# tkonolige/city2ba

Hardware: NVIDIA B200
Metric: camera-point visibility tests/sec (higher is better)
Workload: dtype f64

## Files before the change

city2ba_b200/csrc/c2b_api.cu:

```cuda
#include <algorithm>
#include <charconv>
#include <chrono>
#include <cmath>
#include <cstdlib>
#include <condition_variable>
#include <deque>
#include <mutex>
#include <new>
#include <string>
#include <thread>
#include <vector>

#if defined(__linux__)
#include <cerrno>
#include <fcntl.h>
#include <unistd.h>
#include <sys/mman.h>
#include <sys/stat.h>
#endif

#include "c2b_bal.cuh"
#include "c2b_bal_read.cuh"
#include "c2b_bvh.cuh"
#include "c2b_common.cuh"
// ... 670 lines not shown
}

static void reach_box(const double clo[3], const double chi[3], double max_dist, double lo[3], double hi[3]) {
  for (int k = 0; k < 3; ++k) {
    const double pad = max_dist + 1e-6 * (std::fabs(max_dist) + std::fabs(clo[k]) + std::fabs(chi[k]));
    lo[k] = clo[k] - pad;
    hi[k] = chi[k] + pad;
  }
}

static int build_grid(c2b_ctx *ctx, CtxExtra *x, double max_dist) {
  cudaStream_t st = ctx->stream;
  const uint64_t P = ctx->P;
  C2B_CUDA(cudaStreamSynchronize(st));
  GridDesc g;
  double h = max_dist * x->tun.grid_cell_factor;
  double ext[3];
  for (int k = 0; k < 3; ++k) {
    g.min_c[k] = x->pts_bounds[k];
    g.max_c[k] = x->pts_bounds[3 + k];
    ext[k] = g.max_c[k] - g.min_c[k];
    if (!(ext[k] >= 0.0) || std::isinf(ext[k])) ext[k] = 0.0;
    g.lo[k] = std::isfinite(g.min_c[k]) ? g.min_c[k] : 0.0;
  }
  if (!(h > 0.0) || !std::isfinite(h)) h = 1.0;
  const double max_cells = 4194304.0;
  auto cells_at = [&](double hh) {
    double total = 1.0;
    for (int k = 0; k < 3; ++k) total *= std::min(std::floor(ext[k] / hh) + 1.0, 1e9);
    return total;
  };
  x->grid.hinted = false;
  g.drop = 0;
  for (int k = 0; k < 3; ++k) g.rlo[k] = g.rhi[k] = 0.0;
  bool odd_bounds = false;
  for (int k = 0; k < 3; ++k) odd_bounds = odd_bounds || !std::isfinite(g.min_c[k]) || !std::isfinite(g.max_c[k]);
  if (ctx->C) {
    double clo[3], chi[3], rlo[3], rhi[3];
    C2B_TRY(camera_bbox(ctx, clo, chi));
    reach_box(clo, chi, max_dist, rlo, rhi);
    bool usable = true;
    for (int k = 0; k < 3; ++k) usable = usable && std::isfinite(rlo[k]) && std::isfinite(rhi[k]) && rlo[k] <= rhi[k];
    double frac = 1.0;
    if (usable)
      for (int k = 0; k < 3; ++k) {
        const double a = std::fmax(g.min_c[k], rlo[k]), b = std::fmin(g.max_c[k], rhi[k]);
        if (ext[k] > 0.0) frac *= a <= b ? std::fmin((b - a) / ext[k], 1.0) : 0.0;
      }
    if (usable && (cells_at(h) > max_cells || odd_bounds || frac < 0.7)) {
      for (int k = 0; k < 3; ++k) {
        const double a = std::fmax(g.min_c[k], rlo[k]), b = std::fmin(g.max_c[k], rhi[k]);
        g.lo[k] = a <= b ? a : rlo[k];
        ext[k] = a <= b ? b - a : 0.0;
        g.min_c[k] = g.lo[k];
        g.max_c[k] = a <= b ? b : g.lo[k];
        g.rlo[k] = rlo[k];
        g.rhi[k] = rhi[k];
        x->grid.hint_lo[k] = rlo[k];
        x->grid.hint_hi[k] = rhi[k];
      }
      g.drop = 1;
      x->grid.hinted = true;
    }
  }
  for (;;) {
    double total = 1.0;
    for (int k = 0; k < 3; ++k) {
      double nk = std::floor(ext[k] / h) + 1.0;
      if (nk > 1e9) nk = 1e9;
      g.n[k] = (int)nk;
      total *= nk;
    }
    if (total <= max_cells) break;
    h *= 1.5;
  }
  g.inv_h = 1.0 / h;
  uint64_t n_cells = (uint64_t)g.n[0] * g.n[1] * g.n[2];
  C2B_TRY(ctx->cell_of_pt.ensure(P * 4));
  C2B_TRY(ctx->cell_start.ensure((n_cells + 1) * 4));
  C2B_TRY(ctx->cell_cursor.ensure((n_cells + 1) * 4));
  C2B_TRY(ctx->grid_x.ensure(P * 8));
  C2B_TRY(ctx->grid_y.ensure(P * 8));
  C2B_TRY(ctx->grid_z.ensure(P * 8));
  C2B_TRY(ctx->grid_idx.ensure(P * 4));
  C2B_CUDA(cudaMemsetAsync(ctx->cell_start.p, 0, (n_cells + 1) * 4, st));
  const double *px = ctx->pts.as<double>(), *py = px + P, *pz = py + P;
  k_grid_count<<<blocks_for(P, 256), 256, 0, st>>>(px, py, pz, P, g, ctx->cell_of_pt.as<uint32_t>(),
                                                   ctx->cell_start.as<uint32_t>());
  C2B_KERNEL_CHECK();
  C2B_TRY(exclusive_scan_u32(st, ctx->cell_start.as<uint32_t>(), ctx->cell_start.as<uint32_t>(),
                             n_cells + 1, nullptr, ctx->scan_tmp));
  C2B_CUDA(cudaMemcpyAsync(ctx->cell_cursor.p, ctx->cell_start.p, (n_cells + 1) * 4, cudaMemcpyDeviceToDevice, st));
  k_grid_fill<<<blocks_for(P, 256), 256, 0, st>>>(
      px, py, pz, P, ctx->cell_of_pt.as<uint32_t>(), ctx->cell_cursor.as<uint32_t>(), ctx->grid_x.as<double>(),
      ctx->grid_y.as<double>(), ctx->grid_z.as<double>(), ctx->grid_idx.as<uint32_t>());
  C2B_KERNEL_CHECK();
  x->grid.valid = true;
  x->grid.max_dist = max_dist;
  x->grid.points_version = x->points_version;
  x->grid.desc = g;
  x->grid.n_cells = n_cells;
  return C2B_OK;
}

static int ensure_grid(c2b_ctx *ctx, CtxExtra *x, double max_dist) {
  if (!(ctx->C && ctx->P)) return C2B_OK;
  bool valid = x->grid.valid && x->grid.max_dist == max_dist && x->grid.points_version == x->points_version;
  if (valid && x->grid.hinted && !x->grid_locked) {
    double clo[3], chi[3], rlo[3], rhi[3];
    C2B_TRY(camera_bbox(ctx, clo, chi));
    reach_box(clo, chi, max_dist, rlo, rhi);
    for (int k = 0; k < 3; ++k) valid = valid && rlo[k] >= x->grid.hint_lo[k] && rhi[k] <= x->grid.hint_hi[k];
  }
  if (!valid) C2B_TRY(build_grid(ctx, x, max_dist));
  return C2B_OK;
}

namespace {

void fill_stats(c2b_ctx *ctx, c2b_obs *stats, uint64_t C, uint64_t n_cand, uint64_t pairs_eval,
                uint64_t nodes, uint64_t tris) {
  if (!stats) return;
  memset(stats, 0, sizeof *stats);
  stats->n_cameras = C;
  stats->n_obs = ctx->out_O;
  stats->n_candidates = n_cand;
  stats->pairs_evaluated = pairs_eval;
  stats->nodes_visited = nodes;
  stats->tris_tested = tris;
  auto ms = [&](int a, int b) {
    float t = 0;
    cudaEventElapsedTime(&t, ctx->ev[a], ctx->ev[b]);
    return t;
  };
  stats->ms_prep = ms(EV_H2D, EV_PREP);
  stats->ms_cull = ms(EV_PREP, EV_CULL);
  stats->ms_sort = ms(EV_CULL, EV_SORT);
  stats->ms_traverse = ms(EV_SORT, EV_TRAVERSE);
  stats->ms_compact = ms(EV_TRAVERSE, EV_COMPACT);
  stats->ms_total = ms(EV_START, EV_D2H);
}

int visibility_grid_fused(c2b_ctx *ctx, CtxExtra *x, const c2b_scene *scene, double max_dist,
                          const c2b_vis_options &opt, int pbits, int cbits, c2b_obs *stats) {
  cudaStream_t st = ctx->stream;
  const uint64_t C = ctx->C, P = ctx->P;
  const int sel = ctx->out_sel;
  C2B_TRY(ensure_grid(ctx, x, max_dist));
  C2B_CUDA(cudaEventRecord(ctx->ev[EV_PREP], st));

  C2B_TRY(ctx->counters.ensure(128));
  C2B_TRY(ctx->out_offsets[sel].ensure((C + 1) * 8));
  C2B_CUDA(cudaMemsetAsync(ctx->counters.p, 0, 128, st));
  uint64_t n_cand = 0, pairs_eval = 0, total_obs = 0, nodes = 0, tris_t = 0;
  if (!(C && P)) {
    C2B_CUDA(cudaMemsetAsync(ctx->out_offsets[sel].p, 0, (C + 1) * 8, st));
    for (int e : {EV_CULL, EV_SORT, EV_TRAVERSE, EV_COMPACT, EV_D2H}) C2B_CUDA(cudaEventRecord(ctx->ev[e], st));
    C2B_CUDA(cudaStreamSynchronize(st));
    ctx->out_C = C;
    ctx->out_O = 0;
    x->have_result = true;
    x->res_candidates = 0;
    fill_stats(ctx, stats, C, 0, 0, 0, 0);
    return C2B_OK;
  }

  int parts_log2 = 0;
  {
    const uint64_t warps = (uint64_t)ctx->sm_count * FU_RESIDENT_WARPS;
    if (2 * C <= warps) parts_log2 = 1;
    if (4 * C <= warps) parts_log2 = 2;
    if (x->tun.parts_log2 >= 0) parts_log2 = x->tun.parts_log2;
  }
  const uint64_t slots = C << parts_log2;
  C2B_TRY(ctx->ev_off.ensure((slots + 1) * 4));
  C2B_TRY(ctx->vis_count.ensure((slots + 1) * 4));
  C2B_TRY(ctx->seg_off.ensure((slots + 1) * 4));
  const double *cxp = ctx->cam_center.as<double>();
  const bool mesh = opt.occlusion == C2B_OCC_MESH && scene && scene->n_nodes > 0;
  FusedArgs fa;
  memset(&fa, 0, sizeof fa);
  fa.cams = ctx->cams.as<double>();
  fa.cen_x = cxp;
  fa.cen_y = cxp + C;
  fa.cen_z = cxp + 2 * C;
  fa.C = C;
  fa.gx = ctx->grid_x.as<double>();
  fa.gy = ctx->grid_y.as<double>();
  fa.gz = ctx->grid_z.as<double>();
  fa.gidx = ctx->grid_idx.as<uint32_t>();
  fa.cell_start = ctx->cell_start.as<uint32_t>();
  fa.g = x->grid.desc;
  fa.max_dist = max_dist;
  fa.t_star = exact_sq_threshold(max_dist);
  fa.scene_absmax = scene_abs_max(scene);
  fa.endpoint_guard_rel = opt.endpoint_guard_rel;
  fa.block_length = opt.block_length;
  fa.block_inset = opt.block_inset;
  fa.parts_log2 = parts_log2;
  C2B_TRY(ctx->plan_rows.ensure(C * FU_ROWS * sizeof(uint2)));
  C2B_TRY(ctx->plan_row_count.ensure(C * 4));
  fa.rows = ctx->plan_rows.as<uint2>();
  fa.row_count = ctx->plan_row_count.as<uint32_t>();
  fa.ev_count = ctx->ev_off.as<uint32_t>();
  fa.vis_count = ctx->vis_count.as<uint32_t>();
  fa.counters = ctx->counters.as<unsigned long long>();

  uint32_t *d_total = ctx->counters.as<uint32_t>() + 12;
  uint32_t *d_max = ctx->counters.as<uint32_t>() + 13;
  unsigned long long h_cnt[16];

  cudaStream_t ax = ctx->aux_stream;
  if (mesh) {
    const uint32_t trilist_cap = (uint32_t)x->tun.trilist_cap;
    C2B_TRY(ctx->tri_list.ensure((size_t)C * trilist_cap * 4));
    C2B_TRY(ctx->tri_count.ensure(C * 4));
    float rmax = (float)max_dist;
    if ((double)rmax < max_dist) rmax = std::nextafter(rmax, INFINITY);
    rmax = rmax * (1.0f + 4e-6f);
    fa.nodes = scene->nodes.as<float4>();
    fa.tris = scene->tris.as<float4>();
    fa.n_nodes = (int)scene->n_nodes;
    fa.tri_list = ctx->tri_list.as<uint32_t>();
    fa.tri_count = ctx->tri_count.as<uint32_t>();
    fa.tri_cap = trilist_cap;
    fa.hoist_max = (uint32_t)std::min(x->tun.hoist_max, FU_HOIST);
    fa.packet_bvh = x->tun.packet_bvh;
    const bool tl_warp = x->tun.trilist_warp >= 0 ? x->tun.trilist_warp != 0 : C < 32768;
    C2B_CUDA(cudaEventRecord(ctx->ev_fork, st));
    C2B_CUDA(cudaStreamWaitEvent(ax, ctx->ev_fork, 0));
    if (tl_warp)
      k_cam_trilist_warp<<<blocks_for(C, TL_WARPS), TL_WARPS * 32, 0, ax>>>(
          fa.nodes, fa.n_nodes, fa.cen_x, fa.cen_y, fa.cen_z, C, rmax, fa.scene_absmax, trilist_cap,
          ctx->tri_list.as<uint32_t>(), ctx->tri_count.as<uint32_t>(), fa.counters + 0);
    else
      k_cam_trilist<<<blocks_for(C, 128), 128, 0, ax>>>(fa.nodes, fa.n_nodes, fa.cen_x, fa.cen_y, fa.cen_z, C, rmax,
                                                       fa.scene_absmax, trilist_cap, ctx->tri_list.as<uint32_t>(),
                                                       ctx->tri_count.as<uint32_t>(), fa.counters + 0);
    C2B_KERNEL_CHECK();
    C2B_CUDA(cudaEventRecord(ctx->ev_join, ax));
  }
  k_cam_plan<<<blocks_for(C + 1, 128), 128, 0, st>>>(fa);
  C2B_KERNEL_CHECK();
  C2B_TRY(exclusive_scan_u32(st, fa.ev_count, fa.ev_count, slots + 1, nullptr, ctx->scan_tmp));
  if (mesh) C2B_CUDA(cudaStreamWaitEvent(st, ctx->ev_join, 0));
  const uint64_t max_pairs = x->tun.max_pairs;
  const bool mt = mesh && opt.predicate == C2B_PRED_MT;
  const bool optimistic = x->tun.optimistic && x->memo.valid && !opt.count_traversal && ctx->scratch_idx.cap >= 4 &&
                          ctx->out_idx[sel].cap >= 4 && ctx->out_uv[sel].cap >= 16;
  bool any_overflow = x->memo.any_overflow;
  if (!optimistic) {
    C2B_TRY(read_counters(ctx, h_cnt));
    pairs_eval = h_cnt[1];
    any_overflow = h_cnt[0] != 0;
    if (pairs_eval >= max_pairs)
      return set_error(ERR_TOO_LARGE, "more than 2^32 camera-point pairs inside max_dist in one call; shard the cameras");
    C2B_TRY(ctx->scratch_idx.ensure(std::max<uint64_t>(pairs_eval, 1) * 4));
  }
  fa.scratch_idx = ctx->scratch_idx.as<uint32_t>();
  fa.scratch_cap = ctx->scratch_idx.cap / 4;
  C2B_CUDA(cudaEventRecord(ctx->ev[EV_CULL], st));
  C2B_CUDA(cudaEventRecord(ctx->ev[EV_SORT], st));

  C2B_CUDA(cudaMemsetAsync(ctx->vis_count.p, 0, (slots + 1) * 4, st));
  {
    const unsigned nb = (unsigned)std::min<uint64_t>(blocks_for(slots, FU_WARPS), (uint64_t)ctx->sm_count * 8), nt = FU_WARPS * 32;
    const bool cnt = opt.count_traversal != 0;
    if (mt) {
      k_visibility_fused<FU_OCC_NONE, false, 3, false><<<nb, nt, 0, st>>>(fa);
    } else if (mesh) {
      if (cnt)
        k_visibility_fused<FU_OCC_MESH, true, 3, true><<<nb, nt, 0, st>>>(fa);
      else if (any_overflow)
// ... 2009 lines not shown
```

city2ba_b200/csrc/c2b_common.cuh:

```cuda
#pragma once
#include <cuda_runtime.h>

#include <atomic>
#include <cstdarg>
#include <cstdint>
#include <cstdio>
#include <cstring>
#include <memory>
#include <string>
#include <type_traits>
#include <utility>
#include <vector>
#if defined(__linux__)
#include <sys/syscall.h>
#include <unistd.h>
#endif

#include "../../include/city2ba_cuda.h"

namespace c2b {

inline std::string &last_error_ref() {
  static thread_local std::string s;
  return s;
// ... 138 lines not shown
  template <class T>
  T *as() const {
    return reinterpret_cast<T *>(p);
  }
};

template <class H, cudaError_t (*make)(H *, unsigned), cudaError_t (*destroy)(H)>
class CudaHandle {
 public:
  CudaHandle() = default;
  CudaHandle(CudaHandle &&o) noexcept : h_(std::exchange(o.h_, nullptr)) {}
  CudaHandle &operator=(CudaHandle &&o) noexcept {
    if (this != &o) {
      release();
      h_ = std::exchange(o.h_, nullptr);
    }
    return *this;
  }
  ~CudaHandle() { release(); }
  int create(unsigned flags = 0) {
    release();
    C2B_CUDA(make(&h_, flags));
    return C2B_OK;
  }
  void release() {
    if (h_) destroy(h_);
    h_ = nullptr;
  }
  operator H() const { return h_; }

 private:
  H h_ = nullptr;
};
using Event = CudaHandle<cudaEvent_t, cudaEventCreateWithFlags, cudaEventDestroy>;
using Stream = CudaHandle<cudaStream_t, cudaStreamCreateWithFlags, cudaStreamDestroy>;

static_assert(!std::is_copy_constructible<DevBuf>::value && !std::is_copy_constructible<PinBuf>::value &&
                  !std::is_copy_constructible<Event>::value && !std::is_copy_constructible<Stream>::value,
              "owners of device resources are move-only");

struct CtxExtra;

enum StageEvent {
  EV_START = 0,
  EV_H2D,
  EV_PREP,
  EV_CULL,
  EV_SORT,
  EV_TRAVERSE,
  EV_COMPACT,
  EV_D2H,
  EV_COUNT
};

}

struct c2b_scene {
  int device = 0;
  uint64_t n_tris = 0;
  uint64_t n_nodes = 0;
  float lo[3] = {0, 0, 0}, hi[3] = {0, 0, 0};
  c2b::DevBuf nodes;
  c2b::DevBuf tris;
};

struct c2b_ctx {
  int device = 0;
  int sm_count = 148;
  c2b::Stream stream;
  c2b::Stream copy_stream;
  c2b::Stream aux_stream;
  std::unique_ptr<c2b::CtxExtra> extra;
  c2b::Event ev[c2b::EV_COUNT];

  uint64_t C = 0, P = 0;
  c2b::DevBuf cams_all;
  c2b::DevBuf cams;
  c2b::DevBuf cam_center;
  c2b::DevBuf pts;
  c2b::DevBuf pts_aos;
  c2b::DevBuf stage;
  c2b::PinBuf pin_in;

  c2b::DevBuf cell_of_pt, cell_start, cell_cursor, grid_x, grid_y, grid_z, grid_idx;

  c2b::DevBuf pool_key, pool_uv, cam_count, counters;
  c2b::DevBuf sort_keys[2], sort_vals[2], sort_hist;
  c2b::DevBuf scan_tmp[3];
  uint64_t pool_capacity = 0;

  c2b::DevBuf vis_words, word_prefix;
  c2b::DevBuf out_offsets[2], out_idx[2], out_uv[2];
  int out_sel = 0;
  uint64_t out_C = 0, out_O = 0;
  c2b::Event ev_fork, ev_join;
  c2b::Event ev_ready[2], ev_copied[2];
  c2b::DevBuf misc;
  c2b::DevBuf tri_list, tri_count;
  c2b::DevBuf ev_off, vis_count, seg_off, scratch_idx, plan_rows, plan_row_count;
  int numa_node = -1;

  c2b::DevBuf nz_cams, nz_centers, nz_pts, nz_uv, nz_scratch;
  float noise_ms[3] = {0, 0, 0};

  c2b::DevBuf pr_cams[2], pr_pts[2], pr_off[2], pr_idx[2], pr_uv[2];
  c2b::DevBuf pr_parent, pr_size, pr_cam_cnt, pr_pt_cnt, pr_words, pr_prefix, pr_small;

  c2b::PinBuf h_offsets, h_idx, h_uv, h_small;

  ~c2b_ctx();
};
```

city2ba_b200/csrc/c2b_cull.cuh:

```cuda
#pragma once
#include "c2b_common.cuh"
#include "c2b_math.cuh"

namespace c2b {

struct CullArgs {
  const double *cams;
  const double *cen_x, *cen_y, *cen_z;
  const double *px, *py, *pz;
  uint64_t C, P;
  double t_star;
  double t_cons;
  int pbits;
  uint64_t *pool_key;
  double2 *pool_uv;
  uint32_t *cam_count;
  unsigned long long *counters;
  uint64_t pool_capacity;
};

constexpr uint64_t POOL_SENTINEL = ~0ull;

__global__ void k_cam_prep(const double *__restrict__ cams, uint64_t C, double *__restrict__ cx,
                           double *__restrict__ cy, double *__restrict__ cz) {
// ... 87 lines not shown
#pragma unroll
  for (int k = 0; k < CB_PPT; ++k) {
    pi[k] = (uint64_t)blockIdx.x * (CB_THREADS * CB_PPT) + (uint64_t)k * CB_THREADS + threadIdx.x;
    bool ok = pi[k] < a.P;
    px[k] = ok ? a.px[pi[k]] : 1e300;
    py[k] = ok ? a.py[pi[k]] : 1e300;
    pz[k] = ok ? a.pz[pi[k]] : 1e300;
  }
  __syncthreads();
  uint2 *q = s_q[warp];
  int qn = 0;
  const double tc = a.t_cons;
  for (int j = 0; j < ncam; ++j) {
    const double cx = s_cx[j], cy = s_cy[j], cz = s_cz[j];
    bool pass[CB_PPT];
    bool any = false;
#pragma unroll
    for (int k = 0; k < CB_PPT; ++k) {
      double dx = px[k] - cx, dy = py[k] - cy, dz = pz[k] - cz;
      double d2 = fma(dz, dz, fma(dy, dy, dx * dx));
      pass[k] = d2 < tc;
      any |= pass[k];
    }
    if (__any_sync(0xffffffffu, any)) {
#pragma unroll
      for (int k = 0; k < CB_PPT; ++k) {
        unsigned m = __ballot_sync(0xffffffffu, pass[k]);
        if (m) {
          if (pass[k]) q[qn + __popc(m & ((1u << lane) - 1u))] = make_uint2((uint32_t)(cam0 + j), (uint32_t)pi[k]);
          qn += __popc(m);
          __syncwarp();
          if (qn >= 32) {
            brute_drain(a, q, qn - 32, 32);
            qn -= 32;
            __syncwarp();
          }
        }
      }
    }
  }
  if (qn > 0) brute_drain(a, q, 0, qn);
}

struct GridDesc {
  double lo[3];
  double inv_h;
  int n[3];
  int drop;
  double max_c[3];
  double min_c[3];
  double rlo[3], rhi[3];
};

__device__ __forceinline__ int grid_coord(const GridDesc &g, int k, double x) {
  double t = floor(dmul(dsub(x, g.lo[k]), g.inv_h));
  int c = t < 0.0 ? 0 : (t >= (double)g.n[k] ? g.n[k] - 1 : (int)t);
  if (!(t == t)) c = 0;
  return c;
}

__global__ void __launch_bounds__(256) k_grid_count(const double *__restrict__ px, const double *__restrict__ py,
                                                    const double *__restrict__ pz, uint64_t P, GridDesc g,
                                                    uint32_t *__restrict__ cell_of_pt, uint32_t *__restrict__ cell_count) {
  const uint64_t i = (uint64_t)blockIdx.x * blockDim.x + threadIdx.x;
  const int lane = threadIdx.x & 31;
  uint32_t cell = 0xffffffffu;
  if (i < P) {
    const double x = px[i], y = py[i], z = pz[i];
    const bool out = g.drop && (x < g.rlo[0] || x > g.rhi[0] || y < g.rlo[1] || y > g.rhi[1] || z < g.rlo[2] || z > g.rhi[2]);
    if (!out) {
      int cx = grid_coord(g, 0, x), cy = grid_coord(g, 1, y), cz = grid_coord(g, 2, z);
      cell = ((uint32_t)cz * g.n[1] + cy) * g.n[0] + cx;
    }
    cell_of_pt[i] = cell;
  }
  const unsigned peers = __match_any_sync(0xffffffffu, cell);
  if (cell != 0xffffffffu && lane == __ffs(peers) - 1) atomicAdd(&cell_count[cell], (uint32_t)__popc(peers));
}

__global__ void __launch_bounds__(256) k_grid_fill(const double *__restrict__ px, const double *__restrict__ py,
                                                   const double *__restrict__ pz, uint64_t P,
                                                   const uint32_t *__restrict__ cell_of_pt, uint32_t *__restrict__ cursor,
                                                   double *__restrict__ gx, double *__restrict__ gy,
                                                   double *__restrict__ gz, uint32_t *__restrict__ gidx) {
  const uint64_t i = (uint64_t)blockIdx.x * blockDim.x + threadIdx.x;
  const int lane = threadIdx.x & 31;
  const uint32_t cell = i < P ? cell_of_pt[i] : 0xffffffffu;
  const bool valid = cell != 0xffffffffu;
  double x = 0.0, y = 0.0, z = 0.0;
  if (valid) {
    x = px[i];
    y = py[i];
    z = pz[i];
  }
  const unsigned peers = __match_any_sync(0xffffffffu, cell);
  const int leader = __ffs(peers) - 1;
  uint32_t first = 0;
  if (valid && lane == leader) first = atomicAdd(&cursor[cell], (uint32_t)__popc(peers));
  const uint32_t pos = __shfl_sync(0xffffffffu, first, leader) + __popc(peers & ((1u << lane) - 1u));
  if (valid) {
    gx[pos] = x;
    gy[pos] = y;
    gz[pos] = z;
    gidx[pos] = (uint32_t)i;
  }
}

__global__ void k_pts_bounds_partial(const double *__restrict__ px, const double *__restrict__ py,
                                     const double *__restrict__ pz, uint64_t P,
                                     double *__restrict__ partial ) {
  double lo[3] = {INFINITY, INFINITY, INFINITY}, hi[3] = {-INFINITY, -INFINITY, -INFINITY};
  for (uint64_t i = (uint64_t)blockIdx.x * blockDim.x + threadIdx.x; i < P;
       i += (uint64_t)gridDim.x * blockDim.x) {
    double v[3] = {px[i], py[i], pz[i]};
#pragma unroll
    for (int k = 0; k < 3; ++k) {
      lo[k] = fmin(lo[k], v[k]);
      hi[k] = fmax(hi[k], v[k]);
    }
  }
  __shared__ double s[6][8];
#pragma unroll
  for (int k = 0; k < 3; ++k) {
#pragma unroll
    for (int o = 16; o > 0; o >>= 1) {
      lo[k] = fmin(lo[k], __shfl_xor_sync(0xffffffffu, lo[k], o));
      hi[k] = fmax(hi[k], __shfl_xor_sync(0xffffffffu, hi[k], o));
    }
    if ((threadIdx.x & 31) == 0) {
      s[k][threadIdx.x >> 5] = lo[k];
      s[3 + k][threadIdx.x >> 5] = hi[k];
    }
  }
  __syncthreads();
  if (threadIdx.x < 6) {
    double r = s[threadIdx.x][0];
    for (int w = 1; w < (int)(blockDim.x >> 5); ++w)
      r = threadIdx.x < 3 ? fmin(r, s[threadIdx.x][w]) : fmax(r, s[threadIdx.x][w]);
    partial[6 * (uint64_t)blockIdx.x + threadIdx.x] = r;
  }
}
__global__ void k_pts_bounds_final(const double *__restrict__ partial, int nb, double *__restrict__ out) {
  const int lane = threadIdx.x & 31;
  double lo[3] = {INFINITY, INFINITY, INFINITY}, hi[3] = {-INFINITY, -INFINITY, -INFINITY};
  for (int b = lane; b < nb; b += 32) {
#pragma unroll
    for (int k = 0; k < 3; ++k) {
      lo[k] = fmin(lo[k], partial[6 * b + k]);
      hi[k] = fmax(hi[k], partial[6 * b + 3 + k]);
    }
  }
#pragma unroll
  for (int k = 0; k < 3; ++k) {
#pragma unroll
    for (int o = 16; o > 0; o >>= 1) {
      lo[k] = fmin(lo[k], __shfl_xor_sync(0xffffffffu, lo[k], o));
      hi[k] = fmax(hi[k], __shfl_xor_sync(0xffffffffu, hi[k], o));
    }
  }
  if (lane == 0) {
#pragma unroll
    for (int k = 0; k < 3; ++k) {
      out[k] = lo[k];
      out[3 + k] = hi[k];
    }
  }
}

}
```

city2ba_b200/csrc/c2b_fused.cuh:

```cuda
#pragma once
#include "c2b_common.cuh"
#include "c2b_compact.cuh"
#include "c2b_cull.cuh"
#include "c2b_math.cuh"
#include "c2b_traverse.cuh"

namespace c2b {

struct FusedArgs {
  const double *cams;
  const double *cen_x, *cen_y, *cen_z;
  uint64_t C;
  const double *gx, *gy, *gz;
  const uint32_t *gidx;
  const uint32_t *cell_start;
  GridDesc g;
  double max_dist;
  double t_star;
  const float4 *nodes;
  const float4 *tris;
  int n_nodes;
  float scene_absmax;
  const uint32_t *tri_list;
  const uint32_t *tri_count;
  uint32_t tri_cap;
  uint32_t hoist_max;
  int packet_bvh;
  int endpoint_guard_rel;
  double block_length, block_inset;
  int parts_log2;
  uint2 *rows;
  uint32_t *row_count;
  uint32_t *ev_count;
  uint32_t *scratch_idx;
  uint64_t scratch_cap;
  uint32_t *vis_count;
  unsigned long long *counters;
};
enum { FU_FLAG_SCRATCH = 1, FU_FLAG_NEED_WALK = 2, FU_FLAG_OUT = 4 };

__device__ __forceinline__ bool camera_cell_range(const GridDesc &g, const double cc[3], double max_dist,
                                                  int lo[3], int hi[3]) {
  bool empty = !(max_dist > 0.0);
#pragma unroll
  for (int k = 0; k < 3; ++k) {
    const double eps = dadd(dmul(1e-9, dadd(fabs(cc[k]), fabs(max_dist))), 1e-300);
    const double a0 = dsub(dsub(cc[k], max_dist), eps), a1 = dadd(dadd(cc[k], max_dist), eps);
    if (a0 > g.max_c[k] || a1 < g.min_c[k]) empty = true;
    lo[k] = grid_coord(g, k, a0);
    hi[k] = grid_coord(g, k, a1);
  }
  if (!(cc[0] == cc[0] && cc[1] == cc[1] && cc[2] == cc[2])) empty = true;
  return !empty;
}


__device__ __forceinline__ bool trim_halfspace(const GridDesc &g, double cell_h, double nx, double ny, double nz,
                                               double off, double xr, double mag_floor, double y0, double y1,
                                               double z0, double z1, int &x0, int &x1) {
  const double my = ny == 0.0 ? 0.0 : dmul(ny, ny > 0.0 ? y0 : y1);
  const double mz = nz == 0.0 ? 0.0 : dmul(nz, nz > 0.0 ? z0 : z1);
  const double bmin = dadd(dadd(my, mz), off);
  const double mag = dadd(dadd(dadd(dadd(fabs(my), fabs(mz)), fabs(off)), xr), mag_floor);
  if (bmin == bmin && fabs(bmin) < INFINITY) {
    const double slack = dadd(dmul(1e-9, mag), 1e-300);
    if (xr <= slack) {
      if (bmin > dmul(2.0, slack)) return false;
    } else {
      const double xlim = ddiv(-dsub(bmin, slack), nx);
      if (xlim == xlim) {
        const double xs = dmul(1e-9, dadd(fabs(xlim), cell_h));
        if (nx > 0.0) {
          const double xe = dadd(xlim, xs);
          if (xe < g.lo[0]) return false;
          const int xc = grid_coord(g, 0, xe);
          x1 = xc < x1 ? xc : x1;
        } else {
          const double xe = dsub(xlim, xs);
          if (xe > g.max_c[0]) return false;
          const int xc = grid_coord(g, 0, xe);
          x0 = xc > x0 ? xc : x0;
        }
        if (x0 > x1) return false;
      }
    }
  }
  return true;
}

constexpr int FU_ROWS = 32;
constexpr uint32_t FU_ROWS_MANY = 0xffffffffu;

struct RowRange {
  uint32_t start, end;
};

__device__ __forceinline__ RowRange camera_row(const GridDesc &g, const uint32_t *__restrict__ cell_start,
// ... 1 lines not shown
                                               const int lo[3], const int hi[3], double cell_h, int y, int z) {
  RowRange r{0u, 0u};
  int x0 = lo[0], x1 = hi[0];
  const double sl = dmul(1e-6, cell_h);
  const double y0 = y == 0 ? g.min_c[1] : dsub(dadd(g.lo[1], dmul((double)y, cell_h)), sl);
  const double y1 = y == g.n[1] - 1 ? g.max_c[1] : dadd(dadd(g.lo[1], dmul((double)(y + 1), cell_h)), sl);
  const double z0 = z == 0 ? g.min_c[2] : dsub(dadd(g.lo[2], dmul((double)z, cell_h)), sl);
  const double z1 = z == g.n[2] - 1 ? g.max_c[2] : dadd(dadd(g.lo[2], dmul((double)(z + 1), cell_h)), sl);
  const double reach = dadd(fabs(cc[0]), fabs(max_dist));
  {
    const double dy = fmax(fmax(dsub(y0, cc[1]), dsub(cc[1], y1)), 0.0);
    const double dz = fmax(fmax(dsub(z0, cc[2]), dsub(cc[2], z1)), 0.0);
    const double rem = dsub(dmul(dmul(max_dist, max_dist), 1.000000001), dadd(dmul(dy, dy), dmul(dz, dz)));
    if (rem < 0.0) return r;
    if (rem == rem && rem < INFINITY) {
      const double w = dadd(dmul(dsqrt(rem), 1.000000001), dmul(1e-9, reach));
      const double xa = dsub(cc[0], w), xb = dadd(cc[0], w);
      if (xa > g.max_c[0] || xb < g.min_c[0]) return r;
      const int ca = grid_coord(g, 0, xa), cb = grid_coord(g, 0, xb);
      x0 = ca > x0 ? ca : x0;
      x1 = cb < x1 ? cb : x1;
      if (x0 > x1) return r;
    }
  }
  const double f = c[12];
  const bool planar_image = c[13] == 0.0 && c[14] == 0.0 && fabs(f) < INFINITY;
  double rmax = 0.0;
#pragma unroll
  for (int k = 0; k < 12; ++k) rmax = fmax(rmax, fabs(c[k]));
  const double span = dadd(dadd(dadd(fabs(cc[0]), fabs(cc[1])), fabs(cc[2])), dmul(3.0, fabs(max_dist)));
  const double mag_floor = dmul(dadd(planar_image ? fabs(f) : 0.0, 1.0), dmul(rmax, dadd(span, 1.0)));
  if (!trim_halfspace(g, cell_h, c[2], c[5], c[8], c[11], dmul(fabs(c[2]), reach), mag_floor, y0, y1, z0, z1, x0, x1))
    return r;
  if (planar_image) {
#pragma unroll
    for (int k = 0; k < 4; ++k) {
      const int row = k >> 1;
      const double sf = (k & 1) ? -f : f;
      const double nx = dadd(dmul(sf, c[row]), c[2]), ny = dadd(dmul(sf, c[3 + row]), c[5]);
      const double nz = dadd(dmul(sf, c[6 + row]), c[8]), off = dadd(dmul(sf, c[9 + row]), c[11]);
      if (!trim_halfspace(g, cell_h, nx, ny, nz, off, dmul(fabs(nx), reach), mag_floor, y0, y1, z0, z1, x0, x1))
        return r;
    }
  }
  const uint32_t rowbase = ((uint32_t)z * g.n[1] + y) * g.n[0];
  r.start = cell_start[rowbase + x0];
  r.end = cell_start[rowbase + x1 + 1];
  return r;
}

__device__ __forceinline__ bool cull_predicate(const double *cam, V3 center, V3 p, double t_star) {
  const V3 d{dsub(center.x, p.x), dsub(center.y, p.y), dsub(center.z, p.z)};
  if (!(mag2(d) < t_star)) return false;
  const double pcz = dadd(dadd(dadd(dmul(cam[2], p.x), dmul(cam[5], p.y)), dmul(cam[8], p.z)), cam[11]);
  if (!(pcz <= 0.0)) return false;
  const double pcx = dadd(dadd(dadd(dmul(cam[0], p.x), dmul(cam[3], p.y)), dmul(cam[6], p.z)), cam[9]);
  const double pcy = dadd(dadd(dadd(dmul(cam[1], p.x), dmul(cam[4], p.y)), dmul(cam[7], p.z)), cam[10]);
  const double f = cam[12], k1 = cam[13], k2 = cam[14];
  const double az = fabs(pcz);
  if (az > 1e-30 && az < 1e30) {
    const double iz = (double)__frcp_rn(__double2float_rn(pcz));
    const double a = pcx * iz, b = pcy * iz;
    double ua, va, bu, bv;
    if (k1 == 0.0 && k2 == 0.0) {
      ua = fabs(f * a);
      va = fabs(f * b);
      bu = 2e-6 * ua;
      bv = 2e-6 * va;
    } else {
      const double m2p = a * a + b * b;
      const double r = 1.0 + k1 * m2p + k2 * (m2p * m2p);
      const double rb = 1.0 + fabs(k1) * m2p + fabs(k2) * (m2p * m2p);
      ua = fabs(f * r * a);
      va = fabs(f * r * b);
      bu = 2e-6 * fabs(f * a) * rb;
      bv = 2e-6 * fabs(f * b) * rb;
    }
    if (ua <= 1.0 - bu && va <= 1.0 - bv) return true;
    if (ua > 1.0 + bu || va > 1.0 + bv) return false;
  }
  double u, v;
  project(f, k1, k2, V3{pcx, pcy, pcz}, u, v);
  return u >= -1.0 && u <= 1.0 && v >= -1.0 && v <= 1.0;
}

__device__ __noinline__ RowRange camera_row_call(const GridDesc &g, const uint32_t *__restrict__ cell_start,
                                                 const double *c, const double *cc, double max_dist, const int *lo,
                                                 const int *hi, double cell_h, int y, int z) {
  return camera_row(g, cell_start, c, cc, max_dist, lo, hi, cell_h, y, z);
}

__global__ void __launch_bounds__(128, 5) k_cam_plan(FusedArgs a) {
  const uint64_t cam = (uint64_t)blockIdx.x * blockDim.x + threadIdx.x;
  const int S = 1 << a.parts_log2;
  unsigned long long n0 = 0, n1 = 0, n2 = 0, n3 = 0;
  if (cam < a.C) {
    const double cc[3] = {a.cen_x[cam], a.cen_y[cam], a.cen_z[cam]};
    int lo[3], hi[3];
    a.row_count[cam] = 0u;
    if (camera_cell_range(a.g, cc, a.max_dist, lo, hi)) {
      double c[15];
#pragma unroll
      for (int k = 0; k < 15; ++k) c[k] = a.cams[15 * cam + k];
      const double cell_h = ddiv(1.0, a.g.inv_h);
      const int nrows = (hi[1] - lo[1] + 1) * (hi[2] - lo[2] + 1);
      const bool keep = nrows <= FU_ROWS;
      a.row_count[cam] = keep ? (uint32_t)nrows : FU_ROWS_MANY;
      int ri = 0;
      for (int z = lo[2]; z <= hi[2]; ++z)
        for (int y = lo[1]; y <= hi[1]; ++y, ++ri) {
          const RowRange rr = camera_row(a.g, a.cell_start, c, cc, a.max_dist, lo, hi, cell_h, y, z);
          if (keep) a.rows[cam * FU_ROWS + ri] = make_uint2(rr.start, rr.end);
          if (rr.end > rr.start) {
            const unsigned long long m = rr.end - rr.start;
            int part = 0;
            for (int q = 1; q < S; ++q)
              if (ri >= (nrows * q) >> a.parts_log2) part = q;
            n0 += part == 0 ? m : 0ull;
            n1 += part == 1 ? m : 0ull;
            n2 += part == 2 ? m : 0ull;
            n3 += part == 3 ? m : 0ull;
          }
        }
    }
    uint32_t *out = a.ev_count + (cam << a.parts_log2);
    out[0] = (uint32_t)n0;
    if (S > 1) out[1] = (uint32_t)n1;
    if (S > 2) {
      out[2] = (uint32_t)n2;
      out[3] = (uint32_t)n3;
    }
  }
  if (cam == a.C) a.ev_count[cam << a.parts_log2] = 0u;
  unsigned long long n = n0 + n1 + n2 + n3;
#pragma unroll
  for (int o = 16; o > 0; o >>= 1) n += __shfl_xor_sync(0xffffffffu, n, o);
  if ((threadIdx.x & 31) == 0 && n) atomicAdd(&a.counters[1], n);
}

struct SortWriteArgs {
  const uint32_t *ev_off;
  const uint32_t *seg_off;
  uint64_t C;
  const uint32_t *scratch_idx;
  const double *cams;
  const double *p_aos;
  uint64_t *out_offsets;
  uint32_t *out_idx;
  double2 *out_uv;
  int key_bits;
  int parts_log2;
  uint64_t out_cap;
  unsigned long long *flags;
};

struct CamSlices {
  uint32_t base, n;
  uint32_t sub[4], eo[4];
};
template <bool MULTI>
__device__ __forceinline__ CamSlices cam_slices(const SortWriteArgs &s, uint64_t cam) {
  CamSlices cs;
  if (!MULTI) {
    cs.base = s.seg_off[cam];
    cs.n = s.seg_off[cam + 1] - cs.base;
    cs.sub[0] = 0u;
// ... 340 lines not shown
  }
  for (uint32_t base = 0; base < n_list; base += 32) {
    const uint32_t j = base + lane;
    bool overlap = false;
    int slot = 0;
    if (j < n_list) {
      const uint32_t node = mylist[j];
      const float4 lo = __ldg(&a.nodes[2 * node]);
      const float4 hi = __ldg(&a.nodes[2 * node + 1]);
      overlap = box_meets_packet(pb, lo, hi);
      slot = __float_as_int(hi.w);
    }
    if (COUNT) n_vis += min(32u, n_list - base);
    if (!test_leaf_chunk<COUNT>(a, pb, slot, overlap, ray, am, ox, oy, oz, rec, lane, n_tri)) break;
  }
  return alive && !((am >> lane) & 1u);
}

constexpr int FU_LIFO = 576;

template <bool COUNT>
__device__ __forceinline__ int packet_bvh_hit(const FusedArgs &a, const Ray &ray, bool have, float ox, float oy,
                                              float oz, float4 *region, int lane, unsigned &n_vis,
                                              unsigned &n_tri) {
  const bool alive = have && (ray.tfar >= 0.0f) && (ray.dx == ray.dx) && (ray.dy == ray.dy) && (ray.dz == ray.dz);
  unsigned am = __ballot_sync(0xffffffffu, alive);
  if (am == 0u) return 0;
  const PacketBounds pb = packet_bounds(ray, alive, ox, oy, oz, a.scene_absmax);
  float4 *rec = region;
  uint32_t *pending = reinterpret_cast<uint32_t *>(region + 96);
  uint32_t *lifo = pending + 64;
  int sp = 1, np = 0;
  if (lane == 0) lifo[0] = 0u;
  __syncwarp();
  while (sp > 0 || np > 0) {
    if (sp > 0 && np <= 32) {
      const int take = sp < 32 ? sp : 32;
      const bool mine = lane < take;
      bool leaf = false, inner = false;
      int slot = 0;
      uint32_t node = 0, right = 0;
      if (mine) {
        node = lifo[sp - take + lane];
        const float4 lo = __ldg(&a.nodes[2 * node]);
        const float4 hi = __ldg(&a.nodes[2 * node + 1]);
        if (box_meets_packet(pb, lo, hi)) {
          slot = __float_as_int(hi.w);
          leaf = slot >= 0;
          inner = !leaf;
          right = (uint32_t)(-slot - 1);
        }
      }
      __syncwarp();
      sp -= take;
      if (COUNT) n_vis += take;
      const unsigned lm = __ballot_sync(0xffffffffu, leaf), im = __ballot_sync(0xffffffffu, inner);
      if (sp + 2 * __popc(im) > FU_LIFO) return 2;
      const unsigned lt = (1u << lane) - 1u;
      if (leaf) pending[np + __popc(lm & lt)] = (uint32_t)slot;
      if (inner) {
        const int pos = sp + 2 * __popc(im & lt);
        lifo[pos] = node + 1u;
        lifo[pos + 1] = right;
      }
      np += __popc(lm);
      sp += 2 * __popc(im);
      __syncwarp();
    } else {
      const int cnt = np < 32 ? np : 32;
      const bool want = lane < cnt;
      const int slot = want ? (int)pending[np - cnt + lane] : 0;
      np -= cnt;
      if (!test_leaf_chunk<COUNT>(a, pb, slot, want, ray, am, ox, oy, oz, rec, lane, n_tri)) break;
    }
  }
  return alive && !((am >> lane) & 1u) ? 1 : 0;
}

constexpr int FU_REGION_F4 = 4 * FU_HOIST;

template <bool MESH>
struct alignas(16) FuWarpSmem {
  float4 rec[MESH ? FU_REGION_F4 : 1];
  double cam[16];
  uint32_t stage[FU_STAGE];
};

template <int OCC, bool COUNT, int MIN_CTAS, bool WALK>
__global__ void __launch_bounds__(FU_WARPS * 32, fu_min_ctas(MIN_CTAS)) k_visibility_fused(FusedArgs a) {
  typedef FuWarpSmem<OCC == FU_OCC_MESH> WarpSmem;
  __shared__ WarpSmem s_w[FU_WARPS];
  const int lane = threadIdx.x & 31, warp = threadIdx.x >> 5;
  uint32_t w_s = (uint32_t)__cvta_generic_to_shared(&s_w[warp]);
  asm volatile("" : "+r"(w_s));
  WarpSmem *const w = reinterpret_cast<WarpSmem *>(__cvta_shared_to_generic((size_t)w_s));
  double *const c = w->cam;
  uint32_t *stage = w->stage;
  unsigned long long found_total = 0;
  unsigned n_vis_nodes = 0, n_tri = 0;
  const double cell_h = ddiv(1.0, a.g.inv_h);
  for (;;) {
    unsigned long long ticket = 0;
    if (lane == 0) ticket = atomicAdd(&a.counters[7], 1ull);
    const uint64_t slot = __shfl_sync(0xffffffffu, ticket, 0);
    const uint64_t cam = slot >> a.parts_log2;
    if (cam >= a.C) break;
    const int part = (int)(slot & ((1u << a.parts_log2) - 1u));
    __syncwarp();
    double creg = 0.0;
    if (lane < 15) creg = __ldg(&a.cams[15 * cam + lane]);
    const V3 cen{a.cen_x[cam], a.cen_y[cam], a.cen_z[cam]};
    const uint32_t planned_rows = a.row_count[cam];
    const uint32_t ev0 = a.ev_count[slot], ev1 = a.ev_count[slot + 1];
    const uint2 myrow = a.rows[cam * FU_ROWS + lane];
    uint32_t n_list = 0, l0 = 0, l1 = 0;
    const uint32_t *mylist = nullptr;
    if (OCC == FU_OCC_MESH) {
      n_list = a.tri_count[cam];
      mylist = a.tri_list + cam * a.tri_cap;
      if ((uint32_t)lane < a.tri_cap) l0 = mylist[lane];
      if ((uint32_t)lane + 32u < a.tri_cap) l1 = mylist[lane + 32];
    }
    if (lane < 15) c[lane] = creg;
    __syncwarp();
    const bool misfit = (uint64_t)ev1 > a.scratch_cap || (OCC == FU_OCC_MESH && !WALK && n_list == TRILIST_OVERFLOW);
    if (misfit && lane == 0)
      atomicOr(&a.counters[12], (unsigned long long)((uint64_t)ev1 > a.scratch_cap ? FU_FLAG_SCRATCH : FU_FLAG_NEED_WALK));
    if (planned_rows == 0u || misfit) {
      if (lane == 0) a.vis_count[slot] = 0;
      continue;
    }
    const float ox = d2f(cen.x), oy = d2f(cen.y), oz = d2f(cen.z);
    const bool hoisted = OCC == FU_OCC_MESH && n_list <= a.hoist_max;
    if (hoisted) hoist_records(a, l0, l1, n_list, ox, oy, oz, w->rec, lane);
    uint32_t *out = a.scratch_idx + ev0;
    const uint32_t out_cap = ev1 - ev0;
    uint32_t nvis = 0;
    int qn = 0, head = 0;

    auto resolve = [&](int count) {
      const bool have = lane < count;
      Ray ray;
      ray.ox = ox; ray.oy = oy; ray.oz = oz;
      ray.dx = ray.dy = ray.dz = 1.0f;
      ray.tfar = -1.0f;
      uint32_t pt = 0;
      V3 p{0.0, 0.0, 0.0};
      if (have) {
        const int e = (head + lane) & (FU_STAGE - 1);
        const uint32_t i = stage[e];
        pt = a.gidx[i];
        p = V3{a.gx[i], a.gy[i], a.gz[i]};
        if (OCC == FU_OCC_MESH) ray = make_ray(cen, p, a.endpoint_guard_rel != 0);
      }
      bool occ = false;
      if (OCC == FU_OCC_MESH) {
        if (WALK && n_list == TRILIST_OVERFLOW) {
          const int r = a.packet_bvh ? packet_bvh_hit<COUNT>(a, ray, have, ox, oy, oz, w->rec, lane, n_vis_nodes, n_tri) : 2;
          occ = r == 2 ? warp_any_hit<COUNT>(a.nodes, a.tris, a.n_nodes, ray, have, a.scene_absmax, a.counters)
                       : r == 1;
        } else
          occ = packet_any_hit<COUNT>(a, mylist, n_list, ray, have, ox, oy, oz, w->rec, hoisted, lane, n_vis_nodes, n_tri);
      } else if (OCC == FU_OCC_ANALYTIC) {
        occ = have && hits_building(cen, p, a.block_length, a.block_inset);
      }
      const bool vis = have && !occ;
      const unsigned m = __ballot_sync(0xffffffffu, vis);
      if (vis) {
        const uint32_t pos = nvis + __popc(m & ((1u << lane) - 1u));
        if (pos < out_cap)
          out[pos] = pt;
        else
          a.counters[5] = 1ull;
      }
      nvis += __popc(m);
    };

    int lo[3] = {0, 0, 0}, hi[3] = {0, 0, 0}, ny = 1, nrows = (int)planned_rows;
    double cc[3] = {cen.x, cen.y, cen.z};
    if (planned_rows == FU_ROWS_MANY) {
      camera_cell_range(a.g, cc, a.max_dist, lo, hi);
      ny = hi[1] - lo[1] + 1;
      nrows = ny * (hi[2] - lo[2] + 1);
    }
    const int row0 = (nrows * part) >> a.parts_log2, row1 = (nrows * (part + 1)) >> a.parts_log2;
    for (int rb = planned_rows != FU_ROWS_MANY ? 0 : row0; rb < row1; rb += 32) {
      RowRange rr{0u, 0u};
      const int ri = rb + lane;
      if (ri >= row0 && ri < row1) {
        if (planned_rows != FU_ROWS_MANY) {
          rr.start = myrow.x;
          rr.end = myrow.y;
        } else {
          rr = camera_row_call(a.g, a.cell_start, c, cc, a.max_dist, lo, hi, cell_h, lo[1] + ri % ny, lo[2] + ri / ny);
        }
      }
      unsigned live = __ballot_sync(0xffffffffu, rr.end > rr.start);
      if (live == 0u) continue;
      int j = __ffs(live) - 1;
      live &= live - 1;
      uint32_t base = __shfl_sync(0xffffffffu, rr.start, j), end = __shfl_sync(0xffffffffu, rr.end, j);
      V3 pn{0.0, 0.0, 0.0};
      if (base + lane < end) pn = V3{a.gx[base + lane], a.gy[base + lane], a.gz[base + lane]};
      for (;;) {
        uint32_t nbase = base + 32, nend = end;
        bool more = true;
        if (nbase >= end) {
          if (live) {
            j = __ffs(live) - 1;
            live &= live - 1;
            nbase = __shfl_sync(0xffffffffu, rr.start, j);
            nend = __shfl_sync(0xffffffffu, rr.end, j);
          } else {
            more = false;
          }
        }
        const uint32_t i = base + lane;
        const V3 pcur = pn;
        if (more && nbase + lane < nend) pn = V3{a.gx[nbase + lane], a.gy[nbase + lane], a.gz[nbase + lane]};
        bool pass = false;
        if (i < end) pass = cull_predicate(c, cen, pcur, a.t_star);
        const unsigned m = __ballot_sync(0xffffffffu, pass);
        if (m != 0u) {
          if (pass) {
            const int e = (head + qn + __popc(m & ((1u << lane) - 1u))) & (FU_STAGE - 1);
            stage[e] = i;
          }
          qn += __popc(m);
          __syncwarp();
          if (qn >= 32) {
            resolve(32);
            __syncwarp();
            head = (head + 32) & (FU_STAGE - 1);
            qn -= 32;
            found_total += 32;
          }
        }
        if (!more) break;
        base = nbase;
        end = nend;
      }
    }
    if (qn > 0) {
      resolve(qn);
      found_total += qn;
    }
    nvis = nvis < out_cap ? nvis : out_cap;
    if (lane == 0) a.vis_count[slot] = nvis;
  }
  if (lane == 0) {
    if (found_total) atomicAdd(&a.counters[4], found_total);
    if (COUNT) {
      atomicAdd(&a.counters[2], (unsigned long long)n_vis_nodes);
      atomicAdd(&a.counters[3], (unsigned long long)n_tri);
    }
  }
}

template <int MIN_CTAS, bool MULTI>
__global__ void __launch_bounds__(SW_WARPS * 32, MIN_CTAS) k_sort_write(SortWriteArgs s) {
  __shared__ uint32_t s_sorted[SW_WARPS][SW_WARP_MAX + SW_WARP_MAX / 32];
  __shared__ uint32_t s_hist[SW_WARPS][SW_BINS];
  __shared__ double s_cam[SW_WARPS][16];
  const int lane = threadIdx.x & 31, warp = threadIdx.x >> 5;
  const uint64_t cam = (uint64_t)blockIdx.x * SW_WARPS + warp;
  if (cam >= s.C) return;
  CamSlices cs = cam_slices<MULTI>(s, cam);
  cs.n = __reduce_max_sync(0xffffffffu, cs.n);
  const uint32_t base = cs.base, n = cs.n;
  if (lane == 0) {
    s.out_offsets[cam] = base;
    if (cam == s.C - 1) s.out_offsets[s.C] = s.seg_off[s.C << s.parts_log2];
  }
  if (n == 0 || n > SW_WARP_MAX) return;
  if ((uint64_t)base + n > s.out_cap) {
    if (lane == 0) atomicOr(s.flags, (unsigned long long)FU_FLAG_OUT);
    return;
  }
  uint32_t *sorted = s_sorted[warp];
  if (n <= 128)
    sort_warp_to_smem<4, MULTI>(s, cs, lane, sorted, s_hist[warp]);
  else if (n <= 256)
    sort_warp_to_smem<8, MULTI>(s, cs, lane, sorted, s_hist[warp]);
  else if (n <= 512)
    sort_warp_to_smem<16, MULTI>(s, cs, lane, sorted, s_hist[warp]);
  else if (n <= 768)
    sort_warp_to_smem<24, MULTI>(s, cs, lane, sorted, s_hist[warp]);
  else
    sort_warp_to_smem<32, MULTI>(s, cs, lane, sorted, s_hist[warp]);
  __syncwarp();
  double *crec = s_cam[warp];
  if (lane < 15) crec[lane] = __ldg(&s.cams[15 * cam + lane]);
  __syncwarp();
  uint32_t c_s = (uint32_t)__cvta_generic_to_shared(crec);
  struct Pt {
    uint32_t idx;
    double x, y, z;
  };
  auto gather = [&](uint32_t k) {
    Pt q{0u, 0.0, 0.0, 0.0};
    if (k < n) {
      q.idx = sorted[sw_pad(k)];
      const double *p = s.p_aos + 3 * (uint64_t)q.idx;
      q.x = __ldg(p);
// ... 84 lines not shown
```

Baseline: 293200 billion.

## Add conservative f32 cull prefilter with packed float4 point layout

Stores a packed float4 (x,y,z as f32 plus the point index) per grid point. The hot cull loop now streams these 16-byte records and runs an f32 classifier using per-camera error bounds, computed once per warp, that decide definite inside or outside. Only ambiguous points fall back to the exact f64 predicate. This is meant to cut f64 arithmetic and the three 8-byte loads per candidate on a GPU with weak FP64 throughput. In exchange it adds a 16-byte-per-point buffer, extra work in grid_fill and per-camera setup, and relies on the error bounds being correct to keep results exact.

```diff
diff --git a/city2ba_b200/csrc/c2b_api.cu b/city2ba_b200/csrc/c2b_api.cu
--- a/city2ba_b200/csrc/c2b_api.cu
+++ b/city2ba_b200/csrc/c2b_api.cu
@@ -776,7 +776,7 @@
   C2B_TRY(ctx->grid_x.ensure(P * 8));
   C2B_TRY(ctx->grid_y.ensure(P * 8));
   C2B_TRY(ctx->grid_z.ensure(P * 8));
-  C2B_TRY(ctx->grid_idx.ensure(P * 4));
+  C2B_TRY(ctx->grid_p4.ensure(P * 16));
   C2B_CUDA(cudaMemsetAsync(ctx->cell_start.p, 0, (n_cells + 1) * 4, st));
   const double *px = ctx->pts.as<double>(), *py = px + P, *pz = py + P;
   k_grid_count<<<blocks_for(P, 256), 256, 0, st>>>(px, py, pz, P, g, ctx->cell_of_pt.as<uint32_t>(),
@@ -787,7 +787,7 @@
   C2B_CUDA(cudaMemcpyAsync(ctx->cell_cursor.p, ctx->cell_start.p, (n_cells + 1) * 4, cudaMemcpyDeviceToDevice, st));
   k_grid_fill<<<blocks_for(P, 256), 256, 0, st>>>(
       px, py, pz, P, ctx->cell_of_pt.as<uint32_t>(), ctx->cell_cursor.as<uint32_t>(), ctx->grid_x.as<double>(),
-      ctx->grid_y.as<double>(), ctx->grid_z.as<double>(), ctx->grid_idx.as<uint32_t>());
+      ctx->grid_y.as<double>(), ctx->grid_z.as<double>(), ctx->grid_p4.as<float4>());
   C2B_KERNEL_CHECK();
   x->grid.valid = true;
   x->grid.max_dist = max_dist;
@@ -882,7 +882,7 @@
   fa.gx = ctx->grid_x.as<double>();
   fa.gy = ctx->grid_y.as<double>();
   fa.gz = ctx->grid_z.as<double>();
-  fa.gidx = ctx->grid_idx.as<uint32_t>();
+  fa.gp = ctx->grid_p4.as<float4>();
   fa.cell_start = ctx->cell_start.as<uint32_t>();
   fa.g = x->grid.desc;
   fa.max_dist = max_dist;
diff --git a/city2ba_b200/csrc/c2b_common.cuh b/city2ba_b200/csrc/c2b_common.cuh
--- a/city2ba_b200/csrc/c2b_common.cuh
+++ b/city2ba_b200/csrc/c2b_common.cuh
@@ -244,7 +244,7 @@
   c2b::DevBuf stage;
   c2b::PinBuf pin_in;
 
-  c2b::DevBuf cell_of_pt, cell_start, cell_cursor, grid_x, grid_y, grid_z, grid_idx;
+  c2b::DevBuf cell_of_pt, cell_start, cell_cursor, grid_x, grid_y, grid_z, grid_p4;
 
   c2b::DevBuf pool_key, pool_uv, cam_count, counters;
   c2b::DevBuf sort_keys[2], sort_vals[2], sort_hist;
diff --git a/city2ba_b200/csrc/c2b_cull.cuh b/city2ba_b200/csrc/c2b_cull.cuh
--- a/city2ba_b200/csrc/c2b_cull.cuh
+++ b/city2ba_b200/csrc/c2b_cull.cuh
@@ -193,7 +193,7 @@
                                                    const double *__restrict__ pz, uint64_t P,
                                                    const uint32_t *__restrict__ cell_of_pt, uint32_t *__restrict__ cursor,
                                                    double *__restrict__ gx, double *__restrict__ gy,
-                                                   double *__restrict__ gz, uint32_t *__restrict__ gidx) {
+                                                   double *__restrict__ gz, float4 *__restrict__ gp) {
   const uint64_t i = (uint64_t)blockIdx.x * blockDim.x + threadIdx.x;
   const int lane = threadIdx.x & 31;
   const uint32_t cell = i < P ? cell_of_pt[i] : 0xffffffffu;
@@ -213,7 +213,7 @@
     gx[pos] = x;
     gy[pos] = y;
     gz[pos] = z;
-    gidx[pos] = (uint32_t)i;
+    gp[pos] = make_float4(d2f(x), d2f(y), d2f(z), __uint_as_float((uint32_t)i));
   }
 }
 
diff --git a/city2ba_b200/csrc/c2b_fused.cuh b/city2ba_b200/csrc/c2b_fused.cuh
--- a/city2ba_b200/csrc/c2b_fused.cuh
+++ b/city2ba_b200/csrc/c2b_fused.cuh
@@ -12,7 +12,7 @@
   const double *cen_x, *cen_y, *cen_z;
   uint64_t C;
   const double *gx, *gy, *gz;
-  const uint32_t *gidx;
+  const float4 *gp;
   const uint32_t *cell_start;
   GridDesc g;
   double max_dist;
@@ -180,6 +180,66 @@
   double u, v;
   project(f, k1, k2, V3{pcx, pcy, pcz}, u, v);
   return u >= -1.0 && u <= 1.0 && v >= -1.0 && v <= 1.0;
+}
+
+struct CullF32 {
+  float4 c;
+  float4 rx;
+  float4 ry;
+  float4 rz;
+};
+
+__device__ __noinline__ void cull_f32_constants(const double *cam, V3 cen, double t_star, CullF32 *out) {
+  const double u = 5.9604644775390625e-08, w = 1.1102230246251565e-16;
+  const double cm = fmax(fmax(fabs(cen.x), fabs(cen.y)), fabs(cen.z));
+  double rmax = 0.0;
+  for (int k = 0; k < 12; ++k) rmax = fmax(rmax, fabs(cam[k]));
+  const double f = cam[12];
+  const bool dist_ok = cm <= 1e30 && rmax <= 1e30 && t_star >= 1e-30 && t_star <= 1e30;
+  const bool planar = cam[13] == 0.0 && cam[14] == 0.0 && fabs(f) >= 1e-6 && fabs(f) <= 1e6;
+  float tin = -1.0f, tout = __int_as_float(0x7fffffff), kk = INFINITY;
+  if (dist_ok) {
+    const double a = 2.5 * u, b = 2.5 * u * cm + 1e-37, s3b = 1.7320508075688774 * b * (1.0 + 1e-12);
+    const double r = sqrt(t_star);
+    const double ri = (1.0 - a) * r * (1.0 - 1e-12) - s3b, ro = (1.0 + a) * r * (1.0 + 1e-12) + s3b;
+    if (ri > 0.0) tin = __double2float_rd(ri * ri * (1.0 - 4.0 * u) * (1.0 - 1e-12));
+    if (!(tin >= 1e-30f)) tin = -1.0f;
+    tout = __double2float_ru(ro * ro * (1.0 + 4.0 * u) * (1.0 + 1e-12));
+    if (planar && tin > 0.0f) {
+      const double qb = sqrt((double)tout * (1.0 + 4.0 * u)) * (1.0 + 1e-12);
+      const double L = (qb + s3b) / (1.0 - a) * (1.0 + 1e-12);
+      double e[3], mx[3];
+      for (int row = 0; row < 3; ++row) {
+        const double r0 = cam[row], r1 = cam[3 + row], r2 = cam[6 + row], t = cam[9 + row];
+        const double n1 = fabs(r0) + fabs(r1) + fabs(r2);
+        const double tau = fabs(r0 * cen.x + r1 * cen.y + r2 * cen.z + t) + 4.01 * w * (n1 * cm + fabs(t));
+        const double e64 = 4.01 * w * (n1 * (cm + L) + fabs(t));
+        e[row] = (n1 * (4.02 * u * qb + a * L + b) + tau + e64) * (1.0 + 1e-12);
+        mx[row] = (n1 * L + tau + e64) * (1.0 + 1e-12);
+      }
+      const double af = fabs(f), exy = fmax(e[0], e[1]), xmax = fmax(mx[0], mx[1]);
+      const double k0 = af * exy + u * af * (xmax + exy) + e[2] + 8.0 * w * mx[2];
+      const double kd = (k0 * (1.0 + 2.0 * u) + 1e-37) * (1.0 + 1e-12);
+      if (kd <= 1e30) kk = __double2float_ru(kd);
+    }
+    if (!(kk < INFINITY)) tin = -1.0f;
+  }
+  out->c = make_float4(d2f(cen.x), d2f(cen.y), d2f(cen.z), tin);
+  out->rx = make_float4(d2f(cam[0]), d2f(cam[3]), d2f(cam[6]), tout);
+  out->ry = make_float4(d2f(cam[1]), d2f(cam[4]), d2f(cam[7]), d2f(fabs(f)));
+  out->rz = make_float4(d2f(cam[2]), d2f(cam[5]), d2f(cam[8]), kk);
+}
+
+__device__ __forceinline__ void cull_classify_f32(const CullF32 &k, float4 p, bool &in, bool &out) {
+  const float qx = fsub(p.x, k.c.x), qy = fsub(p.y, k.c.y), qz = fsub(p.z, k.c.z);
+  const float s = ffma(qz, qz, ffma(qy, qy, fmul(qx, qx)));
+  const float xc = ffma(k.rx.z, qz, ffma(k.rx.y, qy, fmul(k.rx.x, qx)));
+  const float yc = ffma(k.ry.z, qz, ffma(k.ry.y, qy, fmul(k.ry.x, qx)));
+  const float zc = ffma(k.rz.z, qz, ffma(k.rz.y, qy, fmul(k.rz.x, qx)));
+  const float hx = ffma(k.ry.w, fabsf(xc), zc), hy = ffma(k.ry.w, fabsf(yc), zc);
+  const float kk = k.rz.w;
+  in = (s < k.c.w) & (hx < -kk) & (hy < -kk);
+  out = (s >= k.rx.w) | ((s < k.rx.w) & ((hx > kk) | (hy > kk)));
 }
 
 __device__ __noinline__ RowRange camera_row_call(const GridDesc &g, const uint32_t *__restrict__ cell_start,
@@ -686,6 +746,7 @@
 template <bool MESH>
 struct alignas(16) FuWarpSmem {
   float4 rec[MESH ? FU_REGION_F4 : 1];
+  CullF32 cf;
   double cam[16];
   uint32_t stage[FU_STAGE];
 };
@@ -726,6 +787,7 @@
       if ((uint32_t)lane + 32u < a.tri_cap) l1 = mylist[lane + 32];
     }
     if (lane < 15) c[lane] = creg;
+    if (lane == 0) cull_f32_constants(&a.cams[15 * cam], cen, a.t_star, &w->cf);
     __syncwarp();
     const bool misfit = (uint64_t)ev1 > a.scratch_cap || (OCC == FU_OCC_MESH && !WALK && n_list == TRILIST_OVERFLOW);
     if (misfit && lane == 0)
@@ -753,7 +815,7 @@
       if (have) {
         const int e = (head + lane) & (FU_STAGE - 1);
         const uint32_t i = stage[e];
-        pt = a.gidx[i];
+        pt = __ldg(reinterpret_cast<const uint32_t *>(a.gp + i) + 3);
         p = V3{a.gx[i], a.gy[i], a.gz[i]};
         if (OCC == FU_OCC_MESH) ray = make_ray(cen, p, a.endpoint_guard_rel != 0);
       }
@@ -804,8 +866,8 @@
       int j = __ffs(live) - 1;
       live &= live - 1;
       uint32_t base = __shfl_sync(0xffffffffu, rr.start, j), end = __shfl_sync(0xffffffffu, rr.end, j);
-      V3 pn{0.0, 0.0, 0.0};
-      if (base + lane < end) pn = V3{a.gx[base + lane], a.gy[base + lane], a.gz[base + lane]};
+      float4 pn = make_float4(0.0f, 0.0f, 0.0f, 0.0f);
+      if (base + lane < end) pn = __ldg(&a.gp[base + lane]);
       for (;;) {
         uint32_t nbase = base + 32, nend = end;
         bool more = true;
@@ -820,10 +882,15 @@
           }
         }
         const uint32_t i = base + lane;
-        const V3 pcur = pn;
-        if (more && nbase + lane < nend) pn = V3{a.gx[nbase + lane], a.gy[nbase + lane], a.gz[nbase + lane]};
+        const float4 pcur = pn;
+        if (more && nbase + lane < nend) pn = __ldg(&a.gp[nbase + lane]);
         bool pass = false;
-        if (i < end) pass = cull_predicate(c, cen, pcur, a.t_star);
+        if (i < end) {
+          bool in, out;
+          cull_classify_f32(w->cf, pcur, in, out);
+          pass = in;
+          if (!(in | out)) pass = cull_predicate(c, cen, V3{a.gx[i], a.gy[i], a.gz[i]}, a.t_star);
+        }
         const unsigned m = __ballot_sync(0xffffffffu, pass);
         if (m != 0u) {
           if (pass) {
```

After: 312000 billion (median of 6 runs). +6.4%, better.
